# aravindr93/mjrl

Measured on AMD Instinct MI355X. Metric: NPG updates/sec (1M-timestep batch, 64x64 MLP), higher is better.
Workload: dtype f32; 1 GPU; BASELINE configs[1]: HalfCheetah-v2 shapes (obs=17, act=6), 64x64 tanh MLP, NPG 10 CG iters, 1M timesteps/batch (1000 traj x 1000), device-resident update; global_batch=1000000, parallelism=dp1 (trajectory shards, one rank sum per CG iteration: none at one rank), cg_iters=10

## Files before the change

### include/mjx.h

```cpp
#ifndef MJX_H
#define MJX_H

#include <stdint.h>

#ifdef __cplusplus
extern "C" {
#endif

typedef struct mjx_ctx mjx_ctx;

#define MJX_OK 0
#define MJX_ERR_ARG (-1)
#define MJX_ERR_STATE (-2)
#define MJX_ERR_UNSUPPORTED (-3)
#define MJX_ERR_NOGPU (-4)

const char* mjx_last_error(void);
int mjx_version(void);
int mjx_device_count(void);

int mjx_process_state(int64_t* out2);

int mjx_create(mjx_ctx** out, int device, int n, int m, const int* hidden, int n_hidden);
void mjx_destroy(mjx_ctx* ctx);
int64_t mjx_num_params(const mjx_ctx* ctx);
int mjx_uses_fused_path(const mjx_ctx* ctx);
int mjx_fused_info(const mjx_ctx* ctx, int32_t* out4);
int mjx_fused_route(int n, int m, const int* hidden, int n_hidden, int32_t* out4);

int mjx_malloc(void** dev_ptr, int64_t bytes);
int mjx_free(void* dev_ptr);
int mjx_memcpy_h2d(void* dst_dev, const void* src_host, int64_t bytes, void* stream);
int mjx_memcpy_d2h(void* dst_host, const void* src_dev, int64_t bytes, void* stream);
int mjx_stream_sync(void* stream);

int mjx_bind_batch(mjx_ctx* ctx, const float* obs, const float* act, const float* adv,
                   int64_t N_local, int64_t N_global);

int mjx_bind_rows(mjx_ctx* ctx, int64_t N_local, int64_t N_global, const float* adv);
int mjx_bind_policy(mjx_ctx* ctx, const float* theta_new, const float* theta_old,
                    const float* tr_new, const float* tr_old, int old_is_new);

int mjx_surr_vpg(mjx_ctx* ctx, float* grad_out, double* scal_out, void* stream);
// ... 161 lines not shown
```

### mjrl_amd/_lib.py

```python
import ctypes
import os

_HERE = os.path.dirname(os.path.abspath(__file__))
LIB_PATH = os.environ.get("MJX_LIB") or os.path.join(_HERE, "csrc", "libmjx.so")

c_void_p, c_int, c_int64, c_float, c_double = ctypes.c_void_p, ctypes.c_int, ctypes.c_int64, ctypes.c_float, ctypes.c_double

ALLREDUCE_FN = ctypes.CFUNCTYPE(c_int, c_void_p, c_void_p, c_int64, c_void_p)
REDUCE_FN = ctypes.CFUNCTYPE(c_int, c_void_p, c_void_p, c_int64, c_int, c_void_p)

PROTOTYPES = {
    "mjx_last_error": (ctypes.c_char_p, []),
    "mjx_version": (c_int, []),
    "mjx_device_count": (c_int, []),
    "mjx_process_state": (c_int, [ctypes.POINTER(c_int64)]),
    "mjx_create": (c_int, [ctypes.POINTER(c_void_p), c_int, c_int, c_int, ctypes.POINTER(c_int), c_int]),
    "mjx_destroy": (None, [c_void_p]),
    "mjx_num_params": (c_int64, [c_void_p]),
    "mjx_uses_fused_path": (c_int, [c_void_p]),
    "mjx_fused_info": (c_int, [c_void_p, ctypes.POINTER(ctypes.c_int32)]),
    "mjx_fused_route": (c_int, [c_int, c_int, ctypes.POINTER(c_int), c_int, ctypes.POINTER(ctypes.c_int32)]),
    "mjx_malloc": (c_int, [ctypes.POINTER(c_void_p), c_int64]),
    "mjx_free": (c_int, [c_void_p]),
    "mjx_memcpy_h2d": (c_int, [c_void_p, c_void_p, c_int64, c_void_p]),
    "mjx_memcpy_d2h": (c_int, [c_void_p, c_void_p, c_int64, c_void_p]),
    "mjx_stream_sync": (c_int, [c_void_p]),
    "mjx_bind_batch": (c_int, [c_void_p, c_void_p, c_void_p, c_void_p, c_int64, c_int64]),
    "mjx_bind_rows": (c_int, [c_void_p, c_int64, c_int64, c_void_p]),
    "mjx_bind_policy": (c_int, [c_void_p, c_void_p, c_void_p, c_void_p, c_void_p, c_int]),
    "mjx_surr_vpg": (c_int, [c_void_p, c_void_p, c_void_p, c_void_p]),
    "mjx_fvp": (c_int, [c_void_p, c_void_p, c_void_p, c_void_p]),
    "mjx_eval_surr_kl": (c_int, [c_void_p, c_void_p, c_void_p]),
    "mjx_cg_solve": (c_int, [c_void_p, c_void_p, c_int, c_float, c_double, c_void_p, c_void_p, c_void_p, c_void_p, c_void_p]),
    "mjx_cg_init": (c_int, [c_void_p, c_void_p, c_void_p]),
    "mjx_cg_p": (c_void_p, [c_void_p]),
    "mjx_cg_step": (c_int, [c_void_p, c_void_p, c_float, c_double, c_void_p]),
# ... 129 lines not shown
```

### mjrl_amd/csrc/fused_host.h

```cpp
#pragma once

namespace mjx {

#define MJX_FUSED_INSTANCES(X)                                                                                                     \
  X(1, 64, 64, 1, 8, 0) X(2, 32, 32, 1, 8, 0) X(3, 64, 64, 1, 16, 0) X(4, 32, 32, 1, 16, 0) X(5, 32, 32, 2, 8, 0) X(6, 32, 32, 2, 32, 0) \
  X(1, 64, 64, 1, 8, 20) X(1, 64, 64, 1, 8, 12) X(1, 64, 64, 1, 8, 8)
#ifdef MJX_PHASE_CLOCK
constexpr bool FUSED_HAS_DBG = false;
#else
constexpr bool FUSED_HAS_DBG = true;
#endif

template <int ID, int H1_, int H2_, int NT1_, int MP_, int NPC_>
struct FusedInst {
  static constexpr int id = ID, H1 = H1_, H2 = H2_, NT1 = NT1_, MP = MP_, NPC = NPC_;
  static constexpr bool has_dbg = FUSED_HAS_DBG && ID == 1 && NPC_ == 0;
  using Layout = FusedLayout<H1_, H2_, NT1_, MP_>;
  using Slab = RawSlab<H1_, H2_, NT1_, MP_, NPC_>;
};
struct FusedKey { int variant, npc, mp; };
#define MJX_X(id, h1, h2, nt1, mp, npc) {id, npc, mp},
constexpr FusedKey FUSED_KEYS[] = {MJX_FUSED_INSTANCES(MJX_X)};
#undef MJX_X
constexpr int fused_max_mp() { int mp = 0; for (const FusedKey& k : FUSED_KEYS) mp = k.mp > mp ? k.mp : mp; return mp; }
// ... 24 lines not shown
      r.variant = I::id; r.bytes = bytes;
    });
  }
  const int NPr = (n + 1 + 3) & ~3;
  for (const FusedKey& k : FUSED_KEYS) if (r.variant && k.variant == r.variant && k.npc == NPr) r.npc = NPr;
  with_fused_instance(r.variant, r.npc, [&](auto inst) {
    using RS = typename decltype(inst)::Slab;
    r.perm.assign(RS::DR, -1);
    if (RS::fill_perm(r.perm.data(), n, m) && reduction_fits(RS::DR, r.bytes)) r.raw_dr = RS::DR;
  });
  return r;
}

inline bool fvp_bf16x3_on() { static const bool on = env_flag("MJX_FVP_BF16X3", true); return on; }
inline bool fvp_bf16x3_r9_on() { static const bool on = env_flag("MJX_FVP_BF16X3_R9", true); return on; }

struct FusedWS {
  int variant = 0, npc = 0;
  int grid = 256;
  int n = 0, m = 0, oS = 0; int64_t d = 0;
  float* partials = nullptr;
  double* spartials = nullptr;
  int raw_dr = 0; int* raw_perm = nullptr;
  int use_hcache = 1;
  float* hcache = nullptr; size_t hcache_bytes = 0, hc_tile = 0;
  bool acts_ok = false, ximg_ok = false; const float* hcache_obs = nullptr; int64_t hcache_rows = 0;
  float* ocache = nullptr; size_t ocache_bytes = 0;
  float* snap = nullptr; size_t snap_bytes = 0;
  bool ocache_ok = false; int64_t ocache_rows = 0;
  unsigned fvp_seq = 0;
// ... 22 lines not shown
  void on_policy() { acts_ok = false; }
  void on_solve() { fvp_seq = 0; }
  void info(int32_t* out4) const { out4[0] = variant; out4[1] = variant ? npc : 0; out4[2] = variant ? raw_dr : 0; out4[3] = variant ? grid : 0; }

  static bool dbg_generic(const FusedArgs& a) { return FUSED_HAS_DBG && a.dbg != nullptr; }
  FusedArgs complete(FusedArgs a) const { a.partials = partials; a.spartials = spartials; a.raw_dr = dbg_generic(a) ? 0 : raw_dr; return a; }
  template <class I, bool DBG>
  int launch(int mode, const FusedArgs& a, hipStream_t st) const {
    constexpr int H1 = I::H1, H2 = I::H2, NT1 = I::NT1, MP = I::MP, NPC = I::NPC;
    using L = typename I::Layout;
    const int nf = NPC ? NPC - 1 : a.n;
    const bool ev2 = (mode == MODE_EVAL) && MP <= 8;
    const bool cached = (mode == MODE_FVP) && a.hcache != nullptr && !DBG;
    constexpr bool BF3_OK = H1 == 64 && H2 == 64 && MP == 8;
    const bool bf3 = BF3_OK && cached && fvp_bf16x3_on() && L(nf, false, true).bytes() <= LDS_MAX;
    const size_t bytes = L(nf, ev2, bf3).bytes();
    void (*k)(FusedArgs) = nullptr;
    if (mode == MODE_VPG) k = k_fused<H1, H2, NT1, MP, MODE_VPG, DBG, NPC>;
    else if (mode == MODE_FVP) k = cached ? k_fused<H1, H2, NT1, MP, MODE_FVP, false, NPC, true> : k_fused<H1, H2, NT1, MP, MODE_FVP, DBG, NPC>;
    else k = k_fused<H1, H2, NT1, MP, MODE_EVAL, false, NPC>;
    if constexpr (BF3_OK) {
      if (bf3) k = fvp_bf16x3_r9_on() ? k_fused<H1, H2, NT1, MP, MODE_FVP, false, NPC, true, true, true> : k_fused<H1, H2, NT1, MP, MODE_FVP, false, NPC, true, true>;
    }
    if (int rc = lds_limit((const void*)k, bytes)) return rc;
    hipLaunchKernelGGL(k, dim3(ev2 ? 2 * grid : grid), dim3(256), bytes, st, a);
    HIPCHK(hipGetLastError());
    return MJX_OK;
  }
  int dispatch(int mode, const FusedArgs& a, hipStream_t st) const {
    const bool dbg = dbg_generic(a);
    int rc = MJX_OK;
    const bool found = with_fused_instance(variant, dbg ? 0 : npc, [&](auto inst) {
      using I = decltype(inst);
      if constexpr (I::has_dbg) { if (dbg) { rc = launch<I, true>(mode, a, st); return; } }
      rc = launch<I, false>(mode, a, st);
    });
    return found ? rc : fail(MJX_ERR_STATE, "no fused variant");
// ... 63 lines not shown
```

### mjrl_amd/csrc/fused_policy.h

```cpp
#pragma once
#include <hip/hip_runtime.h>
#include <stdint.h>

#include <type_traits>
#include <vector>

namespace mjx {

typedef float f32x16 __attribute__((ext_vector_type(16)));
typedef float f32x4 __attribute__((ext_vector_type(4)));
typedef float f32x2 __attribute__((ext_vector_type(2)));

enum { MODE_VPG = 0, MODE_FVP = 1, MODE_EVAL = 2 };

struct FusedArgs {
  const float* obs;
  const float* act;
  const float* adv;
  int64_t N;
  float inv_N;
  const float* thetaA;
  const float* thetaB;
  const float* trA;
  const float* trB;
// ... 295 lines not shown
  }
};

template <int H1, int H2, int NT1, int MP, int MODE, bool DBG = false, int NPC = 0, bool CACHED = false, bool BF3 = false, bool BF3R9 = false>
__global__ __launch_bounds__(256, (MODE == MODE_EVAL && !DBG && MP <= 8) ? 2 : 1) void k_fused(FusedArgs A) {
  using LT = FusedLayout<H1, H2, NT1, MP>;
  constexpr int MT1 = LT::MT1, MT2 = LT::MT2, S2 = LT::S2, S3 = LT::S3, ST = LT::ST;
  constexpr int RA = MP / 2;
  extern __shared__ __attribute__((aligned(16))) float lds[];
  const int tid = threadIdx.x, lane = tid & 63, j = lane & 31, hi = lane >> 5;
  const int wave = __builtin_amdgcn_readfirstlane(tid >> 6);
  const uint32_t himask = hi ? 0xffffffffu : 0u;
  const int n = A.n, m = A.m;
  constexpr bool EV2 = (MODE == MODE_EVAL) && !DBG && MP <= 8;
  constexpr bool XBF3 = (MODE == MODE_FVP) && CACHED && BF3;
  static_assert(!BF3 || (CACHED && MODE == MODE_FVP && H1 == 64 && H2 == 64), "bf16x3: the cached 64 x 64 Fisher-vector product only");
  constexpr bool XR9 = XBF3 && BF3R9;
  static_assert(!BF3R9 || BF3, "bf16x3 R9: an option of the bf16x3 kernel");
  const LT L(NPC ? NPC - 1 : n, EV2, XBF3);
  const int NP = NPC ? NPC : L.NP;
  const int S1 = NP + 2;
  const FlatOff fo(n, m, H1, H2);

  float* slotA = lds;
  float* slotB = lds + L.SLOT;
  float* trs = lds + L.oTR;
  float* ws = lds + L.oWAVES + wave * L.WAVE;
  float* xs = ws + L.oXS;
  float* xT = ws + L.oXT;
  float* d3T = ws + L.oD3;
  float* bufA = ws + L.oBA;
  float* bufB = ws + L.oBB;

  MJX_GSTAMP(16);
// ... 111 lines not shown
      const float osc = ok ? csr[2] : 0.f;
      cst[9 * MP + 2 * a] = ok ? csr[6] : 0.f;
      cst[9 * MP + 2 * a + 1] = osc * (dk * (osc * A.inv_N));
    }
  }
  if (MODE == MODE_EVAL && mism) lds[L.oWAVES] = 1.0f;
  if (MODE == MODE_EVAL && mismx) lds[L.oWAVES + 1] = 1.0f;
  __syncthreads();
  bool use_oc = false, use_xi = false;
  if (MODE == MODE_EVAL && A.ocache) {
    use_oc = (lds[L.oWAVES] == 0.0f);
    use_xi = use_oc && NPC != 0 && A.hcache != nullptr && (lds[L.oWAVES + 1] == 0.0f);
    __syncthreads();
  }
  Pc3 w3p[XBF3 ? MT2 : 1][XBF3 ? MT1 : 1][2];
  if constexpr (XBF3) {
#pragma unroll
    for (int mt = 0; mt < MT2; ++mt)
#pragma unroll
      for (int kb = 0; kb < MT1; ++kb)
#pragma unroll
        for (int s = 0; s < 2; ++s) {
          const float* row = &slotA[L.oW2 + (32 * mt + j) * S2 + 32 * kb + 16 * s + 4 * hi];
          const f32x4 a = *(const f32x4*)row, b = *(const f32x4*)(row + 8);
          const float x[8] = {a.x, a.y, a.z, a.w, b.x, b.y, b.z, b.w};
          w3p[mt][kb][s] = split3(x);
        }
    Pc3 ip[2], vp[2];
#pragma unroll
    for (int e = 0; e < 2; ++e) {
      const int blk = 4 * e + wave, b2 = blk >> 2, kb = (blk >> 1) & 1, s = blk & 1;
      float x[8];
#pragma unroll
      for (int i = 0; i < 8; ++i) x[i] = slotA[L.oW2 + (32 * kb + 16 * s + 8 * (i >> 2) + 4 * hi + (i & 3)) * S2 + 32 * b2 + j];
      ip[e] = split3(x);
      const float* row = &slotB[L.oW2 + (32 * b2 + j) * S2 + 32 * kb + 16 * s + 4 * hi];
      const f32x4 a = *(const f32x4*)row, b = *(const f32x4*)(row + 8);
      const float y[8] = {a.x, a.y, a.z, a.w, b.x, b.y, b.z, b.w};
      vp[e] = split3(y);
    }
    __syncthreads();
    static_assert(LT::F2_IMG == 3 * 8 * 64 * 4, "image: 3 pieces x 8 operand blocks x 64 lanes x 4 dwords");
#pragma unroll
    for (int e = 0; e < 2; ++e)
#pragma unroll
      for (int p = 0; p < 3; ++p) {
        *(u32x4*)&slotA[L.oW2 + ((p * 8 + 4 * e + wave) * 64 + lane) * 4] = ip[e].p[p];
        *(u32x4*)&slotB[L.oW2 + ((p * 8 + 4 * e + wave) * 64 + lane) * 4] = vp[e].p[p];
      }
    __syncthreads();
  }
  float kc3[MP], kcs[MP];
  if (MODE == MODE_FVP) {
#pragma unroll
    for (int a = 0; a < MP; ++a) {
      kc3[a] = __int_as_float(__builtin_amdgcn_readfirstlane(__float_as_int(cst[9 * MP + 2 * a])));
      kcs[a] = __int_as_float(__builtin_amdgcn_readfirstlane(__float_as_int(cst[9 * MP + 2 * a + 1])));
    }
  }
  float kc3r[RA], kcsr[RA];
  if (MODE == MODE_FVP) {
#pragma unroll
    for (int r = 0; r < RA; ++r) { kc3r[r] = cst[9 * MP + 2 * unit_of(r, hi)]; kcsr[r] = cst[9 * MP + 2 * unit_of(r, hi) + 1]; }
// ... 136 lines not shown
  int64_t tile = (int64_t)blockIdx.x * 4 + wave;
  constexpr bool PINNED = XCACHED || (MODE == MODE_VPG && !DBG);
  uint32_t pinA[PINNED ? 4 * MT2 : 1], pinB[PINNED ? 4 * MT1 : 1];
  if constexpr (PINNED) {
#pragma unroll
    for (int g = 0; g < 4 * MT2; ++g) pinA[g] = lds_pin(&bufA[(8 * g + 4 * hi) * ST + j]);
#pragma unroll
    for (int g = 0; g < 4 * MT1; ++g) pinB[g] = lds_pin(&bufB[(8 * g + 4 * hi) * ST + j]);
  }
  constexpr bool PINX = XCACHED && NPC != 0;
  uint32_t pinX[PINX ? (NPC / 4 + 1) / 2 : 1];
  if constexpr (PINX) {
#pragma unroll
    for (int g = 0; g < (NPC / 4 + 1) / 2; ++g) pinX[g] = lds_pin(&xT[(8 * g + 2 * hi) * ST + j]);
  }
  uint32_t pinW[PINNED && !XBF3 ? 4 * MT2 : 1];
  if constexpr (PINNED && !XBF3) {
#pragma unroll
    for (int g = 0; g < 4 * MT2; ++g) pinW[g] = lds_pin(&slotA[L.oW2 + (8 * g + 4 * hi) * S2 + j]);
  }
  float sum_lsA = 0.f, sum_lsB = 0.f;
  if (MODE != MODE_FVP) {
#pragma unroll
    for (int a = 0; a < MP; ++a) { sum_lsA += cst[C_LS * MP + a]; sum_lsB += cst[C_LSB * MP + a]; }
  }
  uint32_t aoff = (uint32_t)(j * m * 4);
  asm volatile("" : "+v"(aoff));
  const bool rev = XCACHED && A.reverse;
  auto ptile = [&](int64_t t) { return rev ? ntiles - 1 - t : t; };
  if constexpr (DIRX) {
    const int f0 = NPC - 4 + 2 * hi;
    onep = f32x2{f0 == n ? 1.0f : 0.f, f0 + 1 == n ? 1.0f : 0.f};
// ... 304 lines not shown
#pragma unroll
          for (int t = 0; t < 4; ++t)
#pragma unroll
            for (int nt = 0; nt < MT1; ++nt) wc8[t][nt] = LDS_AT(pinW[0])[t * S2 + 32 * nt];
        }
      }
      __builtin_amdgcn_sched_barrier(0);
      MJX_STAMP(7);
#pragma unroll
      for (int mt = 0; mt < MT2; ++mt) pk_mul(dl2s[mt], f2s[mt]);
      f32x16 dl1u[MT1];
      float dl2u[MT2][16];
#pragma unroll
      for (int nt = 0; nt < MT1; ++nt) dl1u[nt] = (f32x16)(0.f);
      if constexpr (XBF3) {
        __builtin_amdgcn_sched_barrier(0);
        load_h(ptile((tile + tstride < ntiles) ? tile + tstride : tile));
        const u32x4* img = (const u32x4*)(slotA + L.oW2) + lane;
        constexpr int NG8 = 2 * MT2;
        Pc3 ac = split3_of(dl2s[0], 0), an = ac, bc[MT1], bn[MT1];
#pragma unroll
        for (int nt = 0; nt < MT1; ++nt)
#pragma unroll
          for (int p = 0; p < 3; ++p) bc[nt].p[p] = img[(p * 8 + nt * 4) * 64];
        __builtin_amdgcn_sched_barrier(0);
        SplitGap gap;
#pragma unroll
        for (int g = 0; g < NG8; ++g) {
          const bool nxt = g + 1 < NG8;
          const int kb1 = nxt ? (g + 1) >> 1 : 0, s1 = (g + 1) & 1;
          Split3Tmp sw;
          float xn[8];
#pragma unroll
          for (int e = 0; e < 8; ++e) xn[e] = dl2s[kb1][8 * s1 + e];
#pragma unroll
          for (int i = 0; i < 6 * MT1; ++i) {
            gap.open();
            dl1u[i / 6] = mfma_bf3_step(ac, bc[i / 6], dl1u[i / 6], i % 6);
            mfma_pin(dl1u[i / 6]);
            __builtin_amdgcn_sched_barrier(0);
            if (nxt) {
#pragma unroll
              for (int q = split3_first(i); q < split3_first(i + 1); ++q) split3_step(an, sw, xn, q, gap);
              if (i >= 3 && i < 9) { const int nt = i < 6 ? 1 : 0, p = i % 3; bn[nt].p[p] = img[(p * 8 + (nt * 2 + kb1) * 2 + s1) * 64]; }
            }
            if (g < MT2) {
              const int r0 = i < 3 ? 2 * i : i < 9 ? i + 3 : 2 * i - 6, r1 = i < 3 ? 2 * i + 2 : i < 9 ? i + 4 : 2 * i - 4;
#pragma unroll
              for (int r = r0; r < r1 && r < 16; ++r) LDS_AT(pinA[4 * g + (r >> 2)])[(r & 3) * ST] = dl2s[g][r];
            } else if (i < 3 || i == (nxt ? 9 : 3)) {
              const int nt = g - MT2, qq = i < 3 ? i : 3;
              const f32x4 v = *(const f32x4*)&bufA[(32 * nt + j) * ST + 8 * qq + 4 * hi];
              dl2u[nt][4 * qq] = v.x; dl2u[nt][4 * qq + 1] = v.y; dl2u[nt][4 * qq + 2] = v.z; dl2u[nt][4 * qq + 3] = v.w;
            }
            __builtin_amdgcn_sched_barrier(0);
          }
          ac = an;
#pragma unroll
          for (int nt = 0; nt < MT1; ++nt) bc[nt] = bn[nt];
        }
      } else {
        constexpr int NG = MT2 * 4;
        constexpr int NGH = NG / 2;
        float wc[4][MT1], wn[4][MT1];
        __builtin_amdgcn_sched_barrier(0);
        load_h(ptile((tile + tstride < ntiles) ? tile + tstride : tile));
#pragma unroll
        for (int t = 0; t < 4; ++t)
#pragma unroll
          for (int nt = 0; nt < MT1; ++nt) wc[t][nt] = wc8[t][nt];
#pragma unroll
        for (int g = 0; g < NG; ++g) {
          const int kb = g >> 2, q = g & 3;
          if (g + 1 < NG) {
            const int kb1 = (g + 1) >> 2, q1 = (g + 1) & 3;
// ... 31 lines not shown
            for (int nt = 0; nt < MT1; ++nt) wc[t][nt] = wn[t][nt];
        }
#pragma unroll
        for (int g = 0; g < NG; ++g) {
          if (g + 1 < NG) __builtin_amdgcn_sched_group_barrier(0x100, 2 * MT1, 0);
#pragma unroll
          for (int i = 0; i < 4 * MT1; ++i) {
            __builtin_amdgcn_sched_group_barrier(0x008, 1, 0);
            if (g < NGH) __builtin_amdgcn_sched_group_barrier(0x200, 1, 0);
            else if (i < (4 * MT2 + NGH - 1) / NGH) __builtin_amdgcn_sched_group_barrier(0x100, 1, 0);
          }
        }
      }
      f32x4 bcs[4][MT1];
      if constexpr (XR9) {
        f32x4 hq[4][MT1];
#pragma unroll
        for (int q = 0; q < 2; ++q)
#pragma unroll
          for (int nt = 0; nt < MT1; ++nt) hq[q][nt] = *(const f32x4*)&bufB[(32 * nt + j) * ST + 8 * q + 4 * hi];
        __builtin_amdgcn_sched_barrier(0);
        MJX_STAMP(8);
#pragma unroll
        for (int nt = 0; nt < MT2; ++nt) {
          f32x2 s2 = {dl2u[nt][0], dl2u[nt][1]};
#pragma unroll
          for (int r = 2; r < 16; r += 2) s2 += f32x2{dl2u[nt][r], dl2u[nt][r + 1]};
          sb2[nt] += s2.x + s2.y;
        }
        Pc3 ac[MT2], bc[MT1], an[MT2], bn[MT1];
#pragma unroll
        for (int mt = 0; mt < MT2; ++mt)
#pragma unroll
          for (int k = 0; k < 4; ++k) split3_pair(ac[mt], k, dl2u[mt][2 * k], dl2u[mt][2 * k + 1]);
#pragma unroll
        for (int nt = 0; nt < MT1; ++nt)
#pragma unroll
          for (int k = 0; k < 4; ++k) split3_pair(bc[nt], k, hq[k >> 1][nt][(2 * k) & 3], hq[k >> 1][nt][(2 * k + 1) & 3]);
        __builtin_amdgcn_sched_barrier(0);
#pragma unroll
        for (int s = 0; s < 2; ++s) {
          if (s == 0) {
#pragma unroll
            for (int q = 2; q < 4; ++q)
#pragma unroll
              for (int nt = 0; nt < MT1; ++nt) hq[q][nt] = *(const f32x4*)&bufB[(32 * nt + j) * ST + 8 * q + 4 * hi];
          }
#pragma unroll
          for (int p = 0; p < 6; ++p) {
            const int pa = p == 0 ? 2 : (p == 2 || p == 3) ? 1 : 0, pb = p == 1 ? 2 : (p == 2 || p == 4) ? 1 : 0;
#pragma unroll
            for (int mt = 0; mt < MT2; ++mt)
#pragma unroll
              for (int nt = 0; nt < MT1; ++nt) {
                MJX_MFMA_BF16_ACC(gW2[mt][nt], ac[mt].p[pa], bc[nt].p[pb]);
                const int i = (p * MT2 + mt) * MT1 + nt;
                if (s == 0) {
                  if (i < 4 * (MT2 + MT1)) {
                    const int o = i >> 2, k = i & 3;
                    if (o < MT2) split3_pair(an[o], k, dl2u[o][8 + 2 * k], dl2u[o][8 + 2 * k + 1]);
                    else split3_pair(bn[o - MT2], k, hq[2 + (k >> 1)][o - MT2][(2 * k) & 3], hq[2 + (k >> 1)][o - MT2][(2 * k + 1) & 3]);
                  }
                } else if (i < 4 * MT1) {
                  const int q = i / MT1, n2 = i % MT1;
                  bcs[q][n2] = *(const f32x4*)&bufB[(32 * n2 + j) * ST + 8 * q + 4 * hi];
                }
                __builtin_amdgcn_sched_barrier(0);
              }
          }
          if (s == 0) {
#pragma unroll
            for (int mt = 0; mt < MT2; ++mt) ac[mt] = an[mt];
#pragma unroll
            for (int nt = 0; nt < MT1; ++nt) bc[nt] = bn[nt];
          }
        }
      } else {
#pragma unroll
        for (int nt = 0; nt < MT1; ++nt) bcs[0][nt] = *(const f32x4*)&bufB[(32 * nt + j) * ST + 4 * hi];
        __builtin_amdgcn_sched_barrier(0);
        MJX_STAMP(8);
#pragma unroll
        for (int q = 1; q < 4; ++q)
#pragma unroll
          for (int nt = 0; nt < MT1; ++nt) bcs[q][nt] = *(const f32x4*)&bufB[(32 * nt + j) * ST + 8 * q + 4 * hi];
#pragma unroll
        for (int q = 0; q < 4; ++q) {
#pragma unroll
          for (int t = 0; t < 4; ++t)
#pragma unroll
            for (int mt = 0; mt < MT2; ++mt)
// ... 482 lines not shown
          kl += Nr * cst[C_RD * MP + a] + cst[C_KD * MP + a];
        }
        if (valid && hi == 0) s_kl += (double)kl;
      } else {
        float w = valid ? advv * LR * A.inv_N : 0.f;
        float d3a[MP];
#pragma unroll
        for (int a = 0; a < MP; ++a) {
          if constexpr (HK) d3a[a] = kosc[a >> 2][a & 3] * ((w * z[a]) * kisg[a >> 2][a & 3]);
          else d3a[a] = cst[C_OSC * MP + a] * ((w * z[a]) * cst[C_ISG * MP + a]);
        }
#pragma unroll
        for (int r = 0; r < RA; ++r) {
          d3r[r] = half_select(himask, d3a[unit_of(r, 1)], d3a[unit_of(r, 0)]);
          const float zr = half_select(himask, z[unit_of(r, 1)], z[unit_of(r, 0)]);
          gls[r] += w * (zr * zr - 1.0f);
        }
        if (DBG && A.dbg && blockIdx.x == 0 && wave == 0 && tile == 0 && hi == 0) {
#pragma unroll
          for (int a = 0; a < MP; ++a) A.dbg[2048 * 4 + a * 32 + j] = muv[a];
          A.dbg[2048 * 4 + MP * 32 + j] = llA;
        }
      }
    }

    __builtin_amdgcn_sched_barrier(0);
    if (MODE != MODE_EVAL) {
#pragma unroll
      for (int r = 0; r < RA; ++r) d3T[unit_of(r, hi) * ST + j] = d3r[r];
      if (MODE != MODE_FVP) {
#pragma unroll
// ... 86 lines not shown
#pragma unroll
      for (int r = 0; r < RA; ++r) sb3r[r] += d3r[r];
      if constexpr (!T2L) {
#pragma unroll
      for (int nt = 0; nt < MT2; ++nt) {
        float sacc = 0.f;
#pragma unroll
        for (int r = 0; r < 16; ++r) sacc += dl2u[nt][r];
        sb2[nt] += sacc;
      }
      }
      MJX_STAMP(10);
      f32x16 dl1u[MT1];
#pragma unroll
      for (int nt = 0; nt < MT1; ++nt) dl1u[nt] = (f32x16)(0.f);
      {
        constexpr int NG = MT2 * 4;
        float wc[4][MT1], wn[4][MT1];
        __builtin_amdgcn_sched_barrier(0);
#pragma unroll
        for (int t = 0; t < 4; ++t)
#pragma unroll
          for (int nt = 0; nt < MT1; ++nt) {
            if constexpr (PINNED) wc[t][nt] = LDS_AT(pinW[0])[t * S2 + 32 * nt];
            else wc[t][nt] = slotA[L.oW2 + (4 * hi + t) * S2 + 32 * nt + j];
          }
#pragma unroll
        for (int g = 0; g < NG; ++g) {
          const int kb = g >> 2, q = g & 3;
          if (g + 1 < NG) {
// ... 84 lines not shown
          for (int t = 0; t < 4; ++t)
#pragma unroll
            for (int mt = 0; mt < MT2; ++mt)
#pragma unroll
              for (int nt = 0; nt < MT1; ++nt) MJX_MFMA_ACC(gW2[mt][nt], dl2u[mt][4 * q + t], bc[nt][t]);
#pragma unroll
          for (int nt = 0; nt < MT1; ++nt)
#pragma unroll
            for (int t = 0; t < 4; t += 2) {
              const f32x2 v = mul_1mh2_pair(dl1u[nt][4 * q + t], dl1u[nt][4 * q + t + 1], bc[nt][t], bc[nt][t + 1]);
              dl1u[nt][4 * q + t] = v.x; dl1u[nt][4 * q + t + 1] = v.y;
            }
#pragma unroll
          for (int nt = 0; nt < MT1; ++nt) bc[nt] = bn[nt];
        }
      }
      if (DBG && A.dbg && blockIdx.x == 0 && wave == 0 && tile == 0) {
        float* g = A.dbg + 2048 * 5;
#pragma unroll
        for (int mt = 0; mt < MT2; ++mt)
#pragma unroll
          for (int r = 0; r < 16; ++r) g[(32 * mt + unit_of(r, hi)) * 32 + j] = dl2s[mt][r];
#pragma unroll
        for (int nt = 0; nt < MT1; ++nt)
#pragma unroll
          for (int r = 0; r < 16; ++r) g[2048 + (32 * nt + j) * 32 + unit_of(r, hi)] = dl1u[nt][r];
      }
      MJX_STAMP(12);
      if constexpr (NPC != 0) {
        const float* xrow = &xT[(lane & 3) * ST + 4 * hi];
// ... 207 lines not shown
```

### mjrl_amd/csrc/mjx.hip

```cpp
#include "../../include/mjx.h"

#include <hip/hip_runtime.h>

#include <cmath>
#include <cstdarg>
#include <cstdio>
#include <cstring>
#include <pthread.h>
#include <unistd.h>
#include <atomic>
#include <string>
#include <condition_variable>
#include <functional>
#include <mutex>
#include <thread>
#include <vector>

#include "baseline.h"
#include "dynamics.h"
#include "dyn_fit_ens.h"
#include "fused_policy.h"
#include "policy_fit.h"
#include "rccl_dyn.h"
#include "launch_state.h"
// ... 187 lines not shown
}

void mjx_destroy(mjx_ctx* c) {
  if (!c) return;
  (void)hipSetDevice(c->device);
  (void)mjx_comm_destroy(c);
  c->lw.release();
  c->lwmb.release();
  for (auto& e : c->prof_ev) hipEventDestroy(e);
  c->fz.release();
  hipFree(c->ident_tr);
  hipFree(c->cg_x); hipFree(c->cg_r); hipFree(c->cg_p); hipFree(c->cg_z); hipFree(c->cg_Ap); hipFree(c->ticket); hipFree(c->cg_scal);
  delete c;
}

int64_t mjx_num_params(const mjx_ctx* c) { return c ? c->d : -1; }
int mjx_uses_fused_path(const mjx_ctx* c) { return c ? (c->fz.variant != 0) : 0; }
int mjx_fused_info(const mjx_ctx* c, int32_t* out) {
  if (!c || !out) return fail(MJX_ERR_ARG, "bad arguments");
  c->fz.info(out);
  return MJX_OK;
}
int mjx_fused_route(int n, int m, const int* hidden, int n_hidden, int32_t* out4) {
  if (!out4 || n <= 0 || m <= 0 || n_hidden < 0 || (n_hidden > 0 && !hidden)) return fail(MJX_ERR_ARG, "bad arguments");
  for (int i = 0; i < n_hidden; ++i) if (hidden[i] <= 0) return fail(MJX_ERR_ARG, "bad hidden size");
  const FusedRoute r = fused_route(n, m, std::vector<int>(hidden, hidden + n_hidden));
  out4[0] = r.variant; out4[1] = r.npc; out4[2] = r.raw_dr; out4[3] = (int32_t)r.bytes;
  return MJX_OK;
}

// ... 1360 lines not shown
```

Baseline: 308.0 updates/s.

## Use bf16x3 split MFMA path for the VPG gradient kernel backward pass

Result: no change. 310.6 updates/s (median of 6 runs) (+0.8%).

```diff
diff --git a/include/mjx.h b/include/mjx.h
--- a/include/mjx.h
+++ b/include/mjx.h
@@ -27,6 +27,8 @@
 int mjx_uses_fused_path(const mjx_ctx* ctx);
 int mjx_fused_info(const mjx_ctx* ctx, int32_t* out4);
 int mjx_fused_route(int n, int m, const int* hidden, int n_hidden, int32_t* out4);
+int mjx_k1_bf16x3_route(int n, int m, const int* hidden, int n_hidden, int old_is_new, int debug, int switch_on, int32_t* out4);
+int mjx_fused_layout(int variant, int npc, int n, int eval_only, int bf3, int32_t* out16);
 
 int mjx_malloc(void** dev_ptr, int64_t bytes);
 int mjx_free(void* dev_ptr);
diff --git a/mjrl_amd/_lib.py b/mjrl_amd/_lib.py
--- a/mjrl_amd/_lib.py
+++ b/mjrl_amd/_lib.py
@@ -20,6 +20,8 @@
     "mjx_uses_fused_path": (c_int, [c_void_p]),
     "mjx_fused_info": (c_int, [c_void_p, ctypes.POINTER(ctypes.c_int32)]),
     "mjx_fused_route": (c_int, [c_int, c_int, ctypes.POINTER(c_int), c_int, ctypes.POINTER(ctypes.c_int32)]),
+    "mjx_k1_bf16x3_route": (c_int, [c_int, c_int, ctypes.POINTER(c_int), c_int, c_int, c_int, c_int, ctypes.POINTER(ctypes.c_int32)]),
+    "mjx_fused_layout": (c_int, [c_int, c_int, c_int, c_int, c_int, ctypes.POINTER(ctypes.c_int32)]),
     "mjx_malloc": (c_int, [ctypes.POINTER(c_void_p), c_int64]),
     "mjx_free": (c_int, [c_void_p]),
     "mjx_memcpy_h2d": (c_int, [c_void_p, c_void_p, c_int64, c_void_p]),
diff --git a/mjrl_amd/csrc/fused_bf3_r8.h b/mjrl_amd/csrc/fused_bf3_r8.h
--- /dev/null
+++ b/mjrl_amd/csrc/fused_bf3_r8.h
@@ -0,0 +1,45 @@
+        __builtin_amdgcn_sched_barrier(0);
+        if constexpr (XCACHED) load_h(ptile((tile + tstride < ntiles) ? tile + tstride : tile));
+        const u32x4* img = (const u32x4*)(img8 + L.oW2) + lane;
+        constexpr int NG8 = 2 * MT2;
+        Pc3 ac = split3_of(dl2s[0], 0), an = ac, bc[MT1], bn[MT1];
+#pragma unroll
+        for (int nt = 0; nt < MT1; ++nt)
+#pragma unroll
+          for (int p = 0; p < 3; ++p) bc[nt].p[p] = img[(p * 8 + nt * 4) * 64];
+        __builtin_amdgcn_sched_barrier(0);
+        SplitGap gap;
+#pragma unroll
+        for (int g = 0; g < NG8; ++g) {
+          const bool nxt = g + 1 < NG8;
+          const int kb1 = nxt ? (g + 1) >> 1 : 0, s1 = (g + 1) & 1;
+          Split3Tmp sw;
+          float xn[8];
+#pragma unroll
+          for (int e = 0; e < 8; ++e) xn[e] = dl2s[kb1][8 * s1 + e];
+#pragma unroll
+          for (int i = 0; i < 6 * MT1; ++i) {
+            gap.open();
+            dl1u[i / 6] = mfma_bf3_step(ac, bc[i / 6], dl1u[i / 6], i % 6);
+            mfma_pin(dl1u[i / 6]);
+            __builtin_amdgcn_sched_barrier(0);
+            if (nxt) {
+#pragma unroll
+              for (int q = split3_first(i); q < split3_first(i + 1); ++q) split3_step(an, sw, xn, q, gap);
+              if (i >= 3 && i < 9) { const int nt = i < 6 ? 1 : 0, p = i % 3; bn[nt].p[p] = img[(p * 8 + (nt * 2 + kb1) * 2 + s1) * 64]; }
+            }
+            if (g < MT2) {
+              const int r0 = i < 3 ? 2 * i : i < 9 ? i + 3 : 2 * i - 6, r1 = i < 3 ? 2 * i + 2 : i < 9 ? i + 4 : 2 * i - 4;
+#pragma unroll
+              for (int r = r0; r < r1 && r < 16; ++r) LDS_AT(pinA[4 * g + (r >> 2)])[(r & 3) * ST] = dl2s[g][r];
+            } else if (i < 3 || i == (nxt ? 9 : 3)) {
+              const int nt = g - MT2, qq = i < 3 ? i : 3;
+              const f32x4 v = *(const f32x4*)&bufA[(32 * nt + j) * ST + 8 * qq + 4 * hi];
+              dl2u[nt][4 * qq] = v.x; dl2u[nt][4 * qq + 1] = v.y; dl2u[nt][4 * qq + 2] = v.z; dl2u[nt][4 * qq + 3] = v.w;
+            }
+            __builtin_amdgcn_sched_barrier(0);
+          }
+          ac = an;
+#pragma unroll
+          for (int nt = 0; nt < MT1; ++nt) bc[nt] = bn[nt];
+        }
diff --git a/mjrl_amd/csrc/fused_bf3_r9.h b/mjrl_amd/csrc/fused_bf3_r9.h
--- /dev/null
+++ b/mjrl_amd/csrc/fused_bf3_r9.h
@@ -0,0 +1,61 @@
+        f32x4 hq[4][MT1];
+#pragma unroll
+        for (int q = 0; q < 2; ++q)
+#pragma unroll
+          for (int nt = 0; nt < MT1; ++nt) hq[q][nt] = *(const f32x4*)&bufB[(32 * nt + j) * ST + 8 * q + 4 * hi];
+        __builtin_amdgcn_sched_barrier(0);
+        MJX_STAMP(XCACHED ? 8 : 11);
+#pragma unroll
+        for (int nt = 0; nt < MT2; ++nt) {
+          f32x2 s2 = {dl2u[nt][0], dl2u[nt][1]};
+#pragma unroll
+          for (int r = 2; r < 16; r += 2) s2 += f32x2{dl2u[nt][r], dl2u[nt][r + 1]};
+          sb2[nt] += s2.x + s2.y;
+        }
+        Pc3 ac[MT2], bc[MT1], an[MT2], bn[MT1];
+#pragma unroll
+        for (int mt = 0; mt < MT2; ++mt)
+#pragma unroll
+          for (int k = 0; k < 4; ++k) split3_pair(ac[mt], k, dl2u[mt][2 * k], dl2u[mt][2 * k + 1]);
+#pragma unroll
+        for (int nt = 0; nt < MT1; ++nt)
+#pragma unroll
+          for (int k = 0; k < 4; ++k) split3_pair(bc[nt], k, hq[k >> 1][nt][(2 * k) & 3], hq[k >> 1][nt][(2 * k + 1) & 3]);
+        __builtin_amdgcn_sched_barrier(0);
+#pragma unroll
+        for (int s = 0; s < 2; ++s) {
+          if (s == 0) {
+#pragma unroll
+            for (int q = 2; q < 4; ++q)
+#pragma unroll
+              for (int nt = 0; nt < MT1; ++nt) hq[q][nt] = *(const f32x4*)&bufB[(32 * nt + j) * ST + 8 * q + 4 * hi];
+          }
+#pragma unroll
+          for (int p = 0; p < 6; ++p) {
+            const int pa = p == 0 ? 2 : (p == 2 || p == 3) ? 1 : 0, pb = p == 1 ? 2 : (p == 2 || p == 4) ? 1 : 0;
+#pragma unroll
+            for (int mt = 0; mt < MT2; ++mt)
+#pragma unroll
+              for (int nt = 0; nt < MT1; ++nt) {
+                MJX_MFMA_BF16_ACC(gW2[mt][nt], ac[mt].p[pa], bc[nt].p[pb]);
+                const int i = (p * MT2 + mt) * MT1 + nt;
+                if (s == 0) {
+                  if (i < 4 * (MT2 + MT1)) {
+                    const int o = i >> 2, k = i & 3;
+                    if (o < MT2) split3_pair(an[o], k, dl2u[o][8 + 2 * k], dl2u[o][8 + 2 * k + 1]);
+                    else split3_pair(bn[o - MT2], k, hq[2 + (k >> 1)][o - MT2][(2 * k) & 3], hq[2 + (k >> 1)][o - MT2][(2 * k + 1) & 3]);
+                  }
+                } else if (i < 4 * MT1) {
+                  const int q = i / MT1, n2 = i % MT1;
+                  bcs[q][n2] = *(const f32x4*)&bufB[(32 * n2 + j) * ST + 8 * q + 4 * hi];
+                }
+                __builtin_amdgcn_sched_barrier(0);
+              }
+          }
+          if (s == 0) {
+#pragma unroll
+            for (int mt = 0; mt < MT2; ++mt) ac[mt] = an[mt];
+#pragma unroll
+            for (int nt = 0; nt < MT1; ++nt) bc[nt] = bn[nt];
+          }
+        }
diff --git a/mjrl_amd/csrc/fused_host.h b/mjrl_amd/csrc/fused_host.h
--- a/mjrl_amd/csrc/fused_host.h
+++ b/mjrl_amd/csrc/fused_host.h
@@ -62,6 +62,22 @@
 
 inline bool fvp_bf16x3_on() { static const bool on = env_flag("MJX_FVP_BF16X3", true); return on; }
 inline bool fvp_bf16x3_r9_on() { static const bool on = env_flag("MJX_FVP_BF16X3_R9", true); return on; }
+inline bool k1_bf16x3_on() { static const bool on = env_flag("MJX_K1_BF16X3", true); return on; }
+inline bool k1_bf16x3_serves(int h1, int h2, int mp, int npc, int mode, bool old_is_new, bool debug, size_t bf3_layout_bytes, bool switch_on) {
+  return h1 == 64 && h2 == 64 && mp == 8 && (npc == 8 || npc == 12 || npc == 20) && mode == MODE_VPG && old_is_new && !debug &&
+         bf3_layout_bytes <= LDS_MAX && switch_on;
+}
+inline void k1_bf16x3_route(int n, int m, const std::vector<int>& hid, bool old_is_new, bool debug, int switch_on, int32_t* out4) {
+  const FusedRoute r = fused_route(n, m, hid);
+  out4[0] = 0; out4[1] = r.npc; out4[2] = (int32_t)r.bytes; out4[3] = 0;
+  with_fused_instance(r.variant, debug ? 0 : r.npc, [&](auto inst) {
+    using I = decltype(inst);
+    const int nf = I::NPC ? I::NPC - 1 : n;
+    const size_t fp32 = typename I::Layout(nf).bytes(), bf3 = typename I::Layout(nf, false, true).bytes();
+    const bool on = k1_bf16x3_serves(I::H1, I::H2, I::MP, I::NPC, MODE_VPG, old_is_new, debug, bf3, switch_on < 0 ? k1_bf16x3_on() : switch_on != 0);
+    out4[0] = on ? 1 : 0; out4[1] = I::NPC; out4[2] = (int32_t)(on ? bf3 : fp32); out4[3] = (int32_t)bf3;
+  });
+}
 
 struct FusedWS {
   int variant = 0, npc = 0;
@@ -114,13 +130,15 @@
     const bool cached = (mode == MODE_FVP) && a.hcache != nullptr && !DBG;
     constexpr bool BF3_OK = H1 == 64 && H2 == 64 && MP == 8;
     const bool bf3 = BF3_OK && cached && fvp_bf16x3_on() && L(nf, false, true).bytes() <= LDS_MAX;
-    const size_t bytes = L(nf, ev2, bf3).bytes();
+    const bool k1bf3 = k1_bf16x3_serves(H1, H2, MP, NPC, mode, a.old_is_new != 0, DBG || dbg_generic(a), L(nf, false, true).bytes(), k1_bf16x3_on());
+    const size_t bytes = L(nf, ev2, bf3 || k1bf3).bytes();
     void (*k)(FusedArgs) = nullptr;
     if (mode == MODE_VPG) k = k_fused<H1, H2, NT1, MP, MODE_VPG, DBG, NPC>;
     else if (mode == MODE_FVP) k = cached ? k_fused<H1, H2, NT1, MP, MODE_FVP, false, NPC, true> : k_fused<H1, H2, NT1, MP, MODE_FVP, DBG, NPC>;
     else k = k_fused<H1, H2, NT1, MP, MODE_EVAL, false, NPC>;
     if constexpr (BF3_OK) {
       if (bf3) k = fvp_bf16x3_r9_on() ? k_fused<H1, H2, NT1, MP, MODE_FVP, false, NPC, true, true, true> : k_fused<H1, H2, NT1, MP, MODE_FVP, false, NPC, true, true>;
+      if constexpr (NPC != 0 && !DBG) { if (k1bf3) k = k_fused<H1, H2, NT1, MP, MODE_VPG, false, NPC, false, true, true>; }
     }
     if (int rc = lds_limit((const void*)k, bytes)) return rc;
     hipLaunchKernelGGL(k, dim3(ev2 ? 2 * grid : grid), dim3(256), bytes, st, a);
diff --git a/mjrl_amd/csrc/fused_policy.h b/mjrl_amd/csrc/fused_policy.h
--- a/mjrl_amd/csrc/fused_policy.h
+++ b/mjrl_amd/csrc/fused_policy.h
@@ -333,10 +333,12 @@
   const int n = A.n, m = A.m;
   constexpr bool EV2 = (MODE == MODE_EVAL) && !DBG && MP <= 8;
   constexpr bool XBF3 = (MODE == MODE_FVP) && CACHED && BF3;
-  static_assert(!BF3 || (CACHED && MODE == MODE_FVP && H1 == 64 && H2 == 64), "bf16x3: the cached 64 x 64 Fisher-vector product only");
+  constexpr bool K1BF3 = (MODE == MODE_VPG) && BF3;
+  static_assert(!BF3 || (H1 == 64 && H2 == 64 && ((CACHED && MODE == MODE_FVP) || (K1BF3 && BF3R9 && !CACHED && !DBG && NPC != 0))),
+                "bf16x3: the cached 64 x 64 Fisher-vector product, and K1 of the instances with a compile-time observation width");
   constexpr bool XR9 = XBF3 && BF3R9;
   static_assert(!BF3R9 || BF3, "bf16x3 R9: an option of the bf16x3 kernel");
-  const LT L(NPC ? NPC - 1 : n, EV2, XBF3);
+  const LT L(NPC ? NPC - 1 : n, EV2, XBF3 || K1BF3);
   const int NP = NPC ? NPC : L.NP;
   const int S1 = NP + 2;
   const FlatOff fo(n, m, H1, H2);
@@ -478,7 +480,9 @@
     __syncthreads();
   }
   Pc3 w3p[XBF3 ? MT2 : 1][XBF3 ? MT1 : 1][2];
-  if constexpr (XBF3) {
+  float* const img8 = XBF3 ? slotA : slotB;
+  if constexpr (XBF3 || K1BF3) {
+    if constexpr (XBF3) {
 #pragma unroll
     for (int mt = 0; mt < MT2; ++mt)
 #pragma unroll
@@ -490,6 +494,7 @@
           const float x[8] = {a.x, a.y, a.z, a.w, b.x, b.y, b.z, b.w};
           w3p[mt][kb][s] = split3(x);
         }
+    }
     Pc3 ip[2], vp[2];
 #pragma unroll
     for (int e = 0; e < 2; ++e) {
@@ -498,10 +503,12 @@
 #pragma unroll
       for (int i = 0; i < 8; ++i) x[i] = slotA[L.oW2 + (32 * kb + 16 * s + 8 * (i >> 2) + 4 * hi + (i & 3)) * S2 + 32 * b2 + j];
       ip[e] = split3(x);
-      const float* row = &slotB[L.oW2 + (32 * b2 + j) * S2 + 32 * kb + 16 * s + 4 * hi];
-      const f32x4 a = *(const f32x4*)row, b = *(const f32x4*)(row + 8);
-      const float y[8] = {a.x, a.y, a.z, a.w, b.x, b.y, b.z, b.w};
-      vp[e] = split3(y);
+      if constexpr (XBF3) {
+        const float* row = &slotB[L.oW2 + (32 * b2 + j) * S2 + 32 * kb + 16 * s + 4 * hi];
+        const f32x4 a = *(const f32x4*)row, b = *(const f32x4*)(row + 8);
+        const float y[8] = {a.x, a.y, a.z, a.w, b.x, b.y, b.z, b.w};
+        vp[e] = split3(y);
+      }
     }
     __syncthreads();
     static_assert(LT::F2_IMG == 3 * 8 * 64 * 4, "image: 3 pieces x 8 operand blocks x 64 lanes x 4 dwords");
@@ -509,8 +516,8 @@
     for (int e = 0; e < 2; ++e)
 #pragma unroll
       for (int p = 0; p < 3; ++p) {
-        *(u32x4*)&slotA[L.oW2 + ((p * 8 + 4 * e + wave) * 64 + lane) * 4] = ip[e].p[p];
-        *(u32x4*)&slotB[L.oW2 + ((p * 8 + 4 * e + wave) * 64 + lane) * 4] = vp[e].p[p];
+        *(u32x4*)&img8[L.oW2 + ((p * 8 + 4 * e + wave) * 64 + lane) * 4] = ip[e].p[p];
+        if constexpr (XBF3) *(u32x4*)&slotB[L.oW2 + ((p * 8 + 4 * e + wave) * 64 + lane) * 4] = vp[e].p[p];
       }
     __syncthreads();
   }
@@ -677,8 +684,8 @@
 #pragma unroll
     for (int g = 0; g < (NPC / 4 + 1) / 2; ++g) pinX[g] = lds_pin(&xT[(8 * g + 2 * hi) * ST + j]);
   }
-  uint32_t pinW[PINNED && !XBF3 ? 4 * MT2 : 1];
-  if constexpr (PINNED && !XBF3) {
+  uint32_t pinW[PINNED && !XBF3 && !K1BF3 ? 4 * MT2 : 1];
+  if constexpr (PINNED && !XBF3 && !K1BF3) {
 #pragma unroll
     for (int g = 0; g < 4 * MT2; ++g) pinW[g] = lds_pin(&slotA[L.oW2 + (8 * g + 4 * hi) * S2 + j]);
   }
@@ -1013,51 +1020,7 @@
 #pragma unroll
       for (int nt = 0; nt < MT1; ++nt) dl1u[nt] = (f32x16)(0.f);
       if constexpr (XBF3) {
-        __builtin_amdgcn_sched_barrier(0);
-        load_h(ptile((tile + tstride < ntiles) ? tile + tstride : tile));
-        const u32x4* img = (const u32x4*)(slotA + L.oW2) + lane;
-        constexpr int NG8 = 2 * MT2;
-        Pc3 ac = split3_of(dl2s[0], 0), an = ac, bc[MT1], bn[MT1];
-#pragma unroll
-        for (int nt = 0; nt < MT1; ++nt)
-#pragma unroll
-          for (int p = 0; p < 3; ++p) bc[nt].p[p] = img[(p * 8 + nt * 4) * 64];
-        __builtin_amdgcn_sched_barrier(0);
-        SplitGap gap;
-#pragma unroll
-        for (int g = 0; g < NG8; ++g) {
-          const bool nxt = g + 1 < NG8;
-          const int kb1 = nxt ? (g + 1) >> 1 : 0, s1 = (g + 1) & 1;
-          Split3Tmp sw;
-          float xn[8];
-#pragma unroll
-          for (int e = 0; e < 8; ++e) xn[e] = dl2s[kb1][8 * s1 + e];
-#pragma unroll
-          for (int i = 0; i < 6 * MT1; ++i) {
-            gap.open();
-            dl1u[i / 6] = mfma_bf3_step(ac, bc[i / 6], dl1u[i / 6], i % 6);
-            mfma_pin(dl1u[i / 6]);
-            __builtin_amdgcn_sched_barrier(0);
-            if (nxt) {
-#pragma unroll
-              for (int q = split3_first(i); q < split3_first(i + 1); ++q) split3_step(an, sw, xn, q, gap);
-              if (i >= 3 && i < 9) { const int nt = i < 6 ? 1 : 0, p = i % 3; bn[nt].p[p] = img[(p * 8 + (nt * 2 + kb1) * 2 + s1) * 64]; }
-            }
-            if (g < MT2) {
-              const int r0 = i < 3 ? 2 * i : i < 9 ? i + 3 : 2 * i - 6, r1 = i < 3 ? 2 * i + 2 : i < 9 ? i + 4 : 2 * i - 4;
-#pragma unroll
-              for (int r = r0; r < r1 && r < 16; ++r) LDS_AT(pinA[4 * g + (r >> 2)])[(r & 3) * ST] = dl2s[g][r];
-            } else if (i < 3 || i == (nxt ? 9 : 3)) {
-              const int nt = g - MT2, qq = i < 3 ? i : 3;
-              const f32x4 v = *(const f32x4*)&bufA[(32 * nt + j) * ST + 8 * qq + 4 * hi];
-              dl2u[nt][4 * qq] = v.x; dl2u[nt][4 * qq + 1] = v.y; dl2u[nt][4 * qq + 2] = v.z; dl2u[nt][4 * qq + 3] = v.w;
-            }
-            __builtin_amdgcn_sched_barrier(0);
-          }
-          ac = an;
-#pragma unroll
-          for (int nt = 0; nt < MT1; ++nt) bc[nt] = bn[nt];
-        }
+#include "fused_bf3_r8.h"
       } else {
         constexpr int NG = MT2 * 4;
         constexpr int NGH = NG / 2;
@@ -1119,67 +1082,7 @@
       }
       f32x4 bcs[4][MT1];
       if constexpr (XR9) {
-        f32x4 hq[4][MT1];
-#pragma unroll
-        for (int q = 0; q < 2; ++q)
-#pragma unroll
-          for (int nt = 0; nt < MT1; ++nt) hq[q][nt] = *(const f32x4*)&bufB[(32 * nt + j) * ST + 8 * q + 4 * hi];
-        __builtin_amdgcn_sched_barrier(0);
-        MJX_STAMP(8);
-#pragma unroll
-        for (int nt = 0; nt < MT2; ++nt) {
-          f32x2 s2 = {dl2u[nt][0], dl2u[nt][1]};
-#pragma unroll
-          for (int r = 2; r < 16; r += 2) s2 += f32x2{dl2u[nt][r], dl2u[nt][r + 1]};
-          sb2[nt] += s2.x + s2.y;
-        }
-        Pc3 ac[MT2], bc[MT1], an[MT2], bn[MT1];
-#pragma unroll
-        for (int mt = 0; mt < MT2; ++mt)
-#pragma unroll
-          for (int k = 0; k < 4; ++k) split3_pair(ac[mt], k, dl2u[mt][2 * k], dl2u[mt][2 * k + 1]);
-#pragma unroll
-        for (int nt = 0; nt < MT1; ++nt)
-#pragma unroll
-          for (int k = 0; k < 4; ++k) split3_pair(bc[nt], k, hq[k >> 1][nt][(2 * k) & 3], hq[k >> 1][nt][(2 * k + 1) & 3]);
-        __builtin_amdgcn_sched_barrier(0);
-#pragma unroll
-        for (int s = 0; s < 2; ++s) {
-          if (s == 0) {
-#pragma unroll
-            for (int q = 2; q < 4; ++q)
-#pragma unroll
-              for (int nt = 0; nt < MT1; ++nt) hq[q][nt] = *(const f32x4*)&bufB[(32 * nt + j) * ST + 8 * q + 4 * hi];
-          }
-#pragma unroll
-          for (int p = 0; p < 6; ++p) {
-            const int pa = p == 0 ? 2 : (p == 2 || p == 3) ? 1 : 0, pb = p == 1 ? 2 : (p == 2 || p == 4) ? 1 : 0;
-#pragma unroll
-            for (int mt = 0; mt < MT2; ++mt)
-#pragma unroll
-              for (int nt = 0; nt < MT1; ++nt) {
-                MJX_MFMA_BF16_ACC(gW2[mt][nt], ac[mt].p[pa], bc[nt].p[pb]);
-                const int i = (p * MT2 + mt) * MT1 + nt;
-                if (s == 0) {
-                  if (i < 4 * (MT2 + MT1)) {
-                    const int o = i >> 2, k = i & 3;
-                    if (o < MT2) split3_pair(an[o], k, dl2u[o][8 + 2 * k], dl2u[o][8 + 2 * k + 1]);
-                    else split3_pair(bn[o - MT2], k, hq[2 + (k >> 1)][o - MT2][(2 * k) & 3], hq[2 + (k >> 1)][o - MT2][(2 * k + 1) & 3]);
-                  }
-                } else if (i < 4 * MT1) {
-                  const int q = i / MT1, n2 = i % MT1;
-                  bcs[q][n2] = *(const f32x4*)&bufB[(32 * n2 + j) * ST + 8 * q + 4 * hi];
-                }
-                __builtin_amdgcn_sched_barrier(0);
-              }
-          }
-          if (s == 0) {
-#pragma unroll
-            for (int mt = 0; mt < MT2; ++mt) ac[mt] = an[mt];
-#pragma unroll
-            for (int nt = 0; nt < MT1; ++nt) bc[nt] = bn[nt];
-          }
-        }
+#include "fused_bf3_r9.h"
       } else {
 #pragma unroll
         for (int nt = 0; nt < MT1; ++nt) bcs[0][nt] = *(const f32x4*)&bufB[(32 * nt + j) * ST + 4 * hi];
@@ -1692,7 +1595,8 @@
         for (int r = 0; r < RA; ++r) {
           d3r[r] = half_select(himask, d3a[unit_of(r, 1)], d3a[unit_of(r, 0)]);
           const float zr = half_select(himask, z[unit_of(r, 1)], z[unit_of(r, 0)]);
-          gls[r] += w * (zr * zr - 1.0f);
+          if constexpr (K1BF3) gls[r] = __builtin_fmaf(w, __builtin_fmaf(zr, zr, -1.0f), gls[r]);
+          else gls[r] += w * (zr * zr - 1.0f);
         }
         if (DBG && A.dbg && blockIdx.x == 0 && wave == 0 && tile == 0 && hi == 0) {
 #pragma unroll
@@ -1809,6 +1713,26 @@
       f32x16 dl1u[MT1];
 #pragma unroll
       for (int nt = 0; nt < MT1; ++nt) dl1u[nt] = (f32x16)(0.f);
+      if constexpr (K1BF3) {
+        float dl2u[MT2][16];
+        f32x4 bcs[4][MT1];
+        {
+#include "fused_bf3_r8.h"
+        }
+        {
+#include "fused_bf3_r9.h"
+        }
+#pragma unroll
+        for (int nt = 0; nt < MT1; ++nt)
+#pragma unroll
+          for (int q = 0; q < 4; ++q)
+#pragma unroll
+            for (int t = 0; t < 4; t += 2) {
+              const f32x2 v = mul_1mh2_pair(dl1u[nt][4 * q + t], dl1u[nt][4 * q + t + 1], bcs[q][nt][t], bcs[q][nt][t + 1]);
+              dl1u[nt][4 * q + t] = v.x; dl1u[nt][4 * q + t + 1] = v.y;
+            }
+        __builtin_amdgcn_sched_barrier(0);
+      } else {
       {
         constexpr int NG = MT2 * 4;
         float wc[4][MT1], wn[4][MT1];
@@ -1923,6 +1847,7 @@
 #pragma unroll
           for (int nt = 0; nt < MT1; ++nt) bc[nt] = bn[nt];
         }
+      }
       }
       if (DBG && A.dbg && blockIdx.x == 0 && wave == 0 && tile == 0) {
         float* g = A.dbg + 2048 * 5;
diff --git a/mjrl_amd/csrc/mjx.hip b/mjrl_amd/csrc/mjx.hip
--- a/mjrl_amd/csrc/mjx.hip
+++ b/mjrl_amd/csrc/mjx.hip
@@ -225,6 +225,22 @@
   delete c;
 }
 
+int mjx_k1_bf16x3_route(int n, int m, const int* hidden, int n_hidden, int old_is_new, int debug, int switch_on, int32_t* out4) {
+  if (!out4 || n <= 0 || m <= 0 || n_hidden < 0 || (n_hidden > 0 && !hidden)) return fail(MJX_ERR_ARG, "bad arguments");
+  for (int i = 0; i < n_hidden; ++i) if (hidden[i] <= 0) return fail(MJX_ERR_ARG, "bad hidden size");
+  k1_bf16x3_route(n, m, std::vector<int>(hidden, hidden + n_hidden), old_is_new != 0, debug != 0, switch_on, out4);
+  return MJX_OK;
+}
+int mjx_fused_layout(int variant, int npc, int n, int eval_only, int bf3, int32_t* out16) {
+  if (!out16 || n <= 0) return fail(MJX_ERR_ARG, "bad arguments");
+  const bool found = with_fused_instance(variant, npc, [&](auto inst) {
+    const typename decltype(inst)::Layout L(n, eval_only != 0, bf3 != 0);
+    const int v[16] = {L.oW1, L.oW2, L.oW3, L.oB2, L.oB3, L.SLOT, L.oXS, L.oXT, L.oD3, L.oBA, L.oBB, L.WAVE, L.oTR, L.oCST, L.oWAVES, L.TOTAL};
+    for (int i = 0; i < 16; ++i) out16[i] = v[i];
+  });
+  return found ? MJX_OK : fail(MJX_ERR_ARG, "no such fused instance");
+}
+
 int64_t mjx_num_params(const mjx_ctx* c) { return c ? c->d : -1; }
 int mjx_uses_fused_path(const mjx_ctx* c) { return c ? (c->fz.variant != 0) : 0; }
 int mjx_fused_info(const mjx_ctx* c, int32_t* out) {
```
